# AgnostiqHQ/covalent-ssh-plugin

Hardware: AMD Instinct MI355X
Metric: electrons_per_sec (higher is better)
Workload: dtype n/a; 1 GPU; model=noop-electron-dispatch, global_batch=1, seq_len=0, parallelism=slots1

## Files before the change

### __graft_entry__.py

```python

from __future__ import annotations

import sys
from pathlib import Path

REPO_ROOT = Path(__file__).resolve().parent
if str(REPO_ROOT) not in sys.path:
    sys.path.insert(0, str(REPO_ROOT))


def build() -> None:
    from covalent_ssh_plugin_amd.ops.build import build as build_lib

    lib = build_lib()
    print(f"built {lib}")
    import covalent_ssh_plugin_amd


def smoke() -> None:
    import asyncio
    import ctypes
    import json
    import os
    import tempfile

    import torch

    from covalent_ssh_plugin_amd import SSHExecutor
    from covalent_ssh_plugin_amd.gpu import probe as gpu_probe

    info = gpu_probe.probe(0)
    print("probe:", json.dumps(info))
    assert "gfx950" in info["gcn_arch"], info
    gpu_probe.warmup(0, 50)

    t = torch.randn(1024, 1024, device="cuda:0")
    torch.cuda.synchronize()
    raw = gpu_probe.staged_d2h_bytes(t.data_ptr(), t.numel() * t.element_size())
# ... 58 lines not shown
```

### covalent_ssh_plugin_amd/gpu/probe.py

```python

from __future__ import annotations

import ctypes
import json
import os
from pathlib import Path
from typing import Optional

_LIB_NAME = "libcsp_gpu.so"
_lib: Optional[ctypes.CDLL] = None


class GpuLibError(RuntimeError):
    """The CDNA4 GPU extension is missing or a call into it failed."""


def local_gpu_lib_path() -> str:
    candidate = Path(__file__).resolve().parent.parent / "ops" / _LIB_NAME
    return str(candidate) if candidate.exists() else ""


def load(path: str = "") -> ctypes.CDLL:
    global _lib
    if _lib is not None:
# ... 14 lines not shown
    lib = ctypes.CDLL(lib_path)

    lib.csp_device_count.restype = ctypes.c_int
    lib.csp_probe_json.restype = ctypes.c_int
    lib.csp_probe_json.argtypes = [ctypes.c_int, ctypes.c_char_p, ctypes.c_size_t]
    lib.csp_probe_props_json.restype = ctypes.c_int
    lib.csp_probe_props_json.argtypes = [ctypes.c_int, ctypes.c_char_p, ctypes.c_size_t]
    lib.csp_warmup.restype = ctypes.c_int
    lib.csp_warmup.argtypes = [ctypes.c_int, ctypes.c_int]
    lib.csp_host_alloc.restype = ctypes.c_void_p
    lib.csp_host_alloc.argtypes = [ctypes.c_size_t]
    lib.csp_host_free.restype = ctypes.c_int
    lib.csp_host_free.argtypes = [ctypes.c_void_p]
    lib.csp_staging_get.restype = ctypes.c_void_p
    lib.csp_staging_get.argtypes = [ctypes.c_size_t]
    lib.csp_staging_alloc.restype = ctypes.c_void_p
    lib.csp_staging_alloc.argtypes = [ctypes.c_size_t]
    lib.csp_staging_release_all.restype = ctypes.c_int
    lib.csp_staging_reset.restype = ctypes.c_int
    lib.csp_memcpy_d2h.restype = ctypes.c_int
    lib.csp_memcpy_d2h.argtypes = [ctypes.c_void_p, ctypes.c_void_p, ctypes.c_size_t]
    lib.csp_memcpy_h2d.restype = ctypes.c_int
    lib.csp_memcpy_h2d.argtypes = [ctypes.c_void_p, ctypes.c_void_p, ctypes.c_size_t]
    lib.csp_mem_info.restype = ctypes.c_int
    lib.csp_mem_info.argtypes = [
        ctypes.c_int,
        ctypes.POINTER(ctypes.c_double),
        ctypes.POINTER(ctypes.c_double),
    ]
    lib.csp_last_error.restype = ctypes.c_char_p

    _lib = lib
    return lib


def _check(lib: ctypes.CDLL, rc: int, what: str) -> None:
    if rc != 0:
        err = lib.csp_last_error().decode(errors="replace")
        raise GpuLibError(f"{what} failed (rc={rc}): {err}")


def device_count() -> int:
    lib = load()
    n = lib.csp_device_count()
    if n < 0:
        _check(lib, n, "csp_device_count")
# ... 8 lines not shown


def probe_props(device: int = 0) -> dict:
    lib = load()
    buf = ctypes.create_string_buffer(8192)
    _check(lib, lib.csp_probe_props_json(device, buf, len(buf)), "csp_probe_props_json")
    return json.loads(buf.value.decode())


def mem_info(device: int = 0) -> dict:
    lib = load()
    free_gb = ctypes.c_double()
    total_gb = ctypes.c_double()
    _check(lib, lib.csp_mem_info(device, ctypes.byref(free_gb), ctypes.byref(total_gb)),
           "csp_mem_info")
    return {"hbm_free_gb": free_gb.value, "hbm_total_gb": total_gb.value}


def warmup(device: int = 0, budget_ms: int = 50) -> None:
    lib = load()
    _check(lib, lib.csp_warmup(device, budget_ms), "csp_warmup")


def staged_d2h_bytes(data_ptr: int, nbytes: int) -> bytes:
    lib = load()
    dst = lib.csp_staging_alloc(nbytes)
    if not dst:
        _check(lib, -1, "csp_staging_alloc")
    try:
        _check(
            lib,
            lib.csp_memcpy_d2h(ctypes.c_void_p(dst), ctypes.c_void_p(data_ptr), nbytes),
            "csp_memcpy_d2h",
        )
        return ctypes.string_at(dst, nbytes)
    finally:
        lib.csp_staging_release_all()
```

### covalent_ssh_plugin_amd/ops/build.py

```python

from __future__ import annotations

import os
import shutil
import subprocess
import sys
from pathlib import Path

OPS_DIR = Path(__file__).resolve().parent
SRC = OPS_DIR / "hip" / "csp_gpu.hip"
OUT = OPS_DIR / "libcsp_gpu.so"

HIPCC = shutil.which("hipcc") or "/opt/rocm/bin/hipcc"
ARCH = os.environ.get("PYTORCH_ROCM_ARCH", "gfx950")


def needs_build() -> bool:
    return not OUT.exists() or OUT.stat().st_mtime < SRC.stat().st_mtime


def build(force: bool = False, verbose: bool = True) -> Path:
    if not force and not needs_build():
        return OUT
    cmd = [
        HIPCC,
        f"--offload-arch={ARCH}",
        "-O3",
        "-std=c++17",
        "-fPIC",
        "-shared",
        str(SRC),
        "-o",
        str(OUT),
    ]
    if verbose:
        print("+", " ".join(cmd), file=sys.stderr)
    subprocess.run(cmd, check=True)
    return OUT


if __name__ == "__main__":
    build(force="--force" in sys.argv)
    print(OUT)
```

### covalent_ssh_plugin_amd/ops/hip/csp_gpu.hip

```cpp

#include <hip/hip_runtime.h>
#include <hip/hip_bf16.h>

#include <cstdio>
#include <cstring>
#include <algorithm>
#include <mutex>
#include <vector>
#include <utility>


static thread_local char g_err[512];

static int set_err(const char* what, hipError_t e) {
    snprintf(g_err, sizeof(g_err), "%s: %s", what, hipGetErrorString(e));
    return -1;
}

#define HIP_TRY(expr)                                    \
    do {                                                 \
        hipError_t _e = (expr);                          \
        if (_e != hipSuccess) return set_err(#expr, _e); \
    } while (0)

extern "C" const char* csp_last_error() { return g_err; }


typedef __bf16 bf16x8 __attribute__((ext_vector_type(8)));
// ... 293 lines not shown
    static hipStream_t s = nullptr;
    static std::once_flag once;
    std::call_once(once, [] {
        if (hipStreamCreateWithFlags(&s, hipStreamNonBlocking) != hipSuccess)
            s = nullptr;
    });
    return s;
}

extern "C" int csp_memcpy_d2h(void* dst_host, const void* src_dev, size_t n) {
    hipStream_t s = copy_stream();
    HIP_TRY(hipMemcpyAsync(dst_host, src_dev, n, hipMemcpyDeviceToHost, s));
    HIP_TRY(hipStreamSynchronize(s));
    return 0;
}

extern "C" int csp_memcpy_h2d(void* dst_dev, const void* src_host, size_t n) {
    hipStream_t s = copy_stream();
    HIP_TRY(hipMemcpyAsync(dst_dev, src_host, n, hipMemcpyHostToDevice, s));
    HIP_TRY(hipStreamSynchronize(s));
    return 0;
}

extern "C" int csp_hbm_bench(int device, int variant, size_t bytes, int reps,
                             double* gbps) {
    HIP_TRY(hipSetDevice(device));
    size_t n4 = bytes / sizeof(float4);
    float4 *a = nullptr, *b = nullptr;
    HIP_TRY(hipMalloc(&a, bytes));
    HIP_TRY(hipMalloc(&b, bytes));
    HIP_TRY(hipMemsetAsync(a, 1, bytes));
    float warm_ms = 0.f, ms = 0.f;
    int rc = run_hbm_sweep(a, b, n4, 2, &warm_ms, variant);
    if (rc == 0) rc = run_hbm_sweep(a, b, n4, reps, &ms, variant);
    (void)hipFree(a);
    (void)hipFree(b);
    if (rc != 0) return rc;
    *gbps = (2.0 * (double)bytes * reps / 1.0e9) / ((double)ms / 1000.0);
    return 0;
}

extern "C" int csp_hbm_bench2(int device, int variant, size_t bytes, int reps,
                              int blocks, int pingpong, double* gbps) {
    HIP_TRY(hipSetDevice(device));
    size_t n4 = bytes / sizeof(float4);
    float4 *a = nullptr, *b = nullptr;
// ... 70 lines not shown
```

### covalent_ssh_plugin_amd/remote/stub.py

```python

from __future__ import annotations

import functools
from pathlib import Path
from typing import Optional

_TEMPLATE_PATH = Path(__file__).parent / "stub_template.py"
_WORKER_TEMPLATE_PATH = Path(__file__).parent / "worker_template.py"


@functools.lru_cache(maxsize=2)
def _template_text(path: str) -> str:
    return Path(path).read_text()

DEFAULT_STAGING_THRESHOLD = 64 * 1024 * 1024


def render_stub(
    *,
    remote_result_file: str,
    remote_function_file: str,
    current_remote_workdir: str,
    remote_meta_file: str = "",
    gpu_lib_path: str = "",
    warmup: bool = True,
    staging_threshold: Optional[int] = None,
) -> str:
    text = _template_text(str(_TEMPLATE_PATH))
    thr = DEFAULT_STAGING_THRESHOLD if staging_threshold is None else int(staging_threshold)
    replacements = {
        "__CSP_RESULT_FILE__": remote_result_file,
        "__CSP_FUNCTION_FILE__": remote_function_file,
        "__CSP_WORKDIR__": current_remote_workdir,
        "__CSP_META_FILE__": remote_meta_file,
        "__CSP_GPU_LIB__": gpu_lib_path,
        "__CSP_WARMUP__": repr(bool(warmup)),
        "__CSP_STAGING_THRESHOLD__": str(thr),
    }
    for token, value in replacements.items():
        text = text.replace(token, value)
    return text


@functools.lru_cache(maxsize=64)
def render_worker(
    *,
    gpu_lib_path: str = "",
    warmup: bool = True,
    staging_threshold: Optional[int] = None,
    idle_timeout: float = 0.0,
    isolate: bool = False,
    isolate_preload: str = "torch",
    telemetry_every: int = 0,
) -> str:
    text = _template_text(str(_WORKER_TEMPLATE_PATH))
    thr = DEFAULT_STAGING_THRESHOLD if staging_threshold is None else int(staging_threshold)
    replacements = {
        "__CSP_GPU_LIB__": gpu_lib_path,
        "__CSP_WARMUP__": repr(bool(warmup)),
        "__CSP_STAGING_THRESHOLD__": str(thr),
        "__CSP_IDLE_TIMEOUT__": repr(float(idle_timeout)),
        "__CSP_ISOLATE__": repr(bool(isolate)),
        "__CSP_ISOLATE_PRELOAD__": str(isolate_preload),
        "__CSP_TELEMETRY_EVERY__": str(int(telemetry_every)),
    }
    for token, value in replacements.items():
        text = text.replace(token, value)
    return text
```

### covalent_ssh_plugin_amd/remote/worker_template.py

```python


import json
import os
import struct
import sys
import time

GPU_LIB = "__CSP_GPU_LIB__"
DO_WARMUP = bool(__CSP_WARMUP__)
STAGING_THRESHOLD = int(__CSP_STAGING_THRESHOLD__)
IDLE_TIMEOUT = float(__CSP_IDLE_TIMEOUT__)
ISOLATE = bool(__CSP_ISOLATE__)
ISOLATE_PRELOAD = "__CSP_ISOLATE_PRELOAD__"
TELEMETRY_EVERY = int(__CSP_TELEMETRY_EVERY__)
_last_mem = None

if GPU_LIB:
    GPU_LIB = os.path.abspath(os.path.expanduser(GPU_LIB))


def _resolve_gpu_slot():
    slot = os.environ.get("CSP_GPU_SLOT")
    if slot is None:
        return None
    ambient = os.environ.get("HIP_VISIBLE_DEVICES") or ""
    ids = [x for x in ambient.split(",") if x.strip() != ""]
    if ids:
        os.environ["HIP_VISIBLE_DEVICES"] = ids[int(slot) % len(ids)]
    else:
        os.environ["HIP_VISIBLE_DEVICES"] = slot
    return slot


# ... 28 lines not shown
    if importlib.util.find_spec("torch") is None:
        return
    import torch

    if torch.cuda.is_available():
        torch.cuda.init()


def _load_gpu_lib():
    import ctypes

    _ensure_torch_runtime_first()

    lib = ctypes.CDLL(GPU_LIB)
    lib.csp_probe_json.restype = ctypes.c_int
    lib.csp_probe_json.argtypes = [ctypes.c_int, ctypes.c_char_p, ctypes.c_size_t]
    lib.csp_warmup.restype = ctypes.c_int
    lib.csp_warmup.argtypes = [ctypes.c_int, ctypes.c_int]
    lib.csp_staging_alloc.restype = ctypes.c_void_p
    lib.csp_staging_alloc.argtypes = [ctypes.c_size_t]
    lib.csp_staging_release_all.restype = ctypes.c_int
    lib.csp_memcpy_d2h.restype = ctypes.c_int
    lib.csp_memcpy_d2h.argtypes = [ctypes.c_void_p, ctypes.c_void_p, ctypes.c_size_t]
    lib.csp_mem_info.restype = ctypes.c_int
    lib.csp_mem_info.argtypes = [
        ctypes.c_int,
        ctypes.POINTER(ctypes.c_double),
        ctypes.POINTER(ctypes.c_double),
    ]
    lib.csp_last_error.restype = ctypes.c_char_p
    return lib


def _sample_hbm():
    global _last_mem
    if _gpu_lib is None:
        return
    import ctypes

    free_gb = ctypes.c_double()
    total_gb = ctypes.c_double()
    if _gpu_lib.csp_mem_info(0, ctypes.byref(free_gb), ctypes.byref(total_gb)) == 0:
        _last_mem = {
            "hbm_free_gb": round(free_gb.value, 2),
            "hbm_total_gb": round(total_gb.value, 2),
            "sampled_at_serial": _served,
# ... 2 lines not shown

def _prologue():
    global _gpu_lib, _gpu_info
    import ctypes

    _gpu_lib = _load_gpu_lib()
    buf = ctypes.create_string_buffer(8192)
    rc = _gpu_lib.csp_probe_json(0, buf, len(buf))
    if rc != 0:
        raise RuntimeError(
            "csp_probe_json failed: %s"
            % _gpu_lib.csp_last_error().decode(errors="replace")
        )
    _gpu_info = json.loads(buf.value.decode())
    if DO_WARMUP:
        rc = _gpu_lib.csp_warmup(0, 50)
        if rc != 0:
            raise RuntimeError(
                "csp_warmup failed: %s"
                % _gpu_lib.csp_last_error().decode(errors="replace")
            )


def _stage_result(result, stats, buffers, buffer_meta):
    if "torch" not in sys.modules:
        return result
    import ctypes

    import torch

    lib = _gpu_lib
    if lib is None and GPU_LIB and os.path.exists(GPU_LIB):
        try:
            lib = _load_gpu_lib()
        except Exception:
            lib = None

    def emit_buffer(view, keepalive, dtype, shape):
        buffers.append((view, keepalive))
        buffer_meta.append(
            {"dtype": str(dtype).replace("torch.", ""), "shape": list(shape)}
        )
        return ("__csp_tensor_buffer_v1__", len(buffers) - 1)

    def to_host(t):
        stats["tensors"] += 1
        nbytes = t.numel() * t.element_size()
        stats["bytes"] += nbytes
        if nbytes < STAGING_THRESHOLD:
            return t.cpu() if t.is_cuda else t
        if t.is_cuda:
            if lib is None:
                raise RuntimeError(
                    "CUDA tensor result but the CDNA4 staging library is "
                    "not available on this GPU host"
                )
            src_t = t.contiguous()
            torch.cuda.synchronize()
            dst = lib.csp_staging_alloc(nbytes)
            if not dst:
                raise RuntimeError("csp_staging_alloc failed")
            rc = lib.csp_memcpy_d2h(
                ctypes.c_void_p(dst), ctypes.c_void_p(src_t.data_ptr()), nbytes
            )
            if rc != 0:
                raise RuntimeError("csp_memcpy_d2h failed")
            view = (ctypes.c_char * nbytes).from_address(dst)
            stats["pinned_tensors"] += 1
            stats["mode"] = "pinned"
            return emit_buffer(view, None, src_t.dtype, src_t.shape)
        src_t = t.contiguous()
        view = (ctypes.c_char * nbytes).from_address(src_t.data_ptr())
        if stats["mode"] != "pinned":
            stats["mode"] = "cpu-oob"
        return emit_buffer(view, src_t, src_t.dtype, src_t.shape)

    def walk(obj):
        if isinstance(obj, torch.Tensor):
            return to_host(obj)
        if isinstance(obj, dict):
            return {k: walk(v) for k, v in obj.items()}
        if isinstance(obj, tuple):
            vals = [walk(v) for v in obj]
            return type(obj)(*vals) if hasattr(obj, "_fields") else tuple(vals)
        if isinstance(obj, list):
            return [walk(v) for v in obj]
        return obj

    return walk(result)


def _read_frame(fd, idle_timeout=0.0):
    if idle_timeout > 0:
# ... 135 lines not shown
    _served += 1
    serial = _served
    r, w = os.pipe()
    pid = os.fork()
    if pid == 0:
        os.close(r)
        try:
            import ctypes

            libc = ctypes.CDLL(None, use_errno=True)
            libc.prctl(1, 9, 0, 0, 0)
        except Exception:
            pass
        wrote_reply = False
        try:
            if GPU_LIB and GPU_SLOT is not None and DO_WARMUP:
                _prologue()
            result_blob, meta, buffers = _serve_one(request)
            meta["isolated"] = True
            meta["served"] = serial
            _write_frame(w, pickle.dumps(("R1", result_blob, meta, len(buffers))))
            wrote_reply = True
            for view, _keep in buffers:
                _write_frame(w, view)
        except BaseException as e:
            if not wrote_reply:
                try:
                    blob = pickle.dumps(
                        (None, RuntimeError(f"isolated task failed: {e!r}"))
                    )
                    _write_frame(
                        w,
                        pickle.dumps(
                            ("R1", blob, {"phases_ms": {}, "isolated": True}, 0)
                        ),
                    )
                except BaseException:
                    pass
        os._exit(0)

    os.close(w)
    relayed = 0
    expected = None
    while True:
        frame = _read_frame(r)
        if frame is None or frame == b"":
            break
# ... 46 lines not shown
        sys.exit(3)

    while True:
        frame = _read_frame(0, idle_timeout=IDLE_TIMEOUT)
        if frame is None or frame == b"":
            break
        request = pickle.loads(frame)
        n_arg_bufs = len(request.get("arg_buffers") or [])
        if n_arg_bufs:
            frames = []
            for _ in range(n_arg_bufs):
                f = _read_frame(0)
                if f is None:
                    return
                frames.append(bytearray(f))
            request["_arg_buffer_frames"] = frames
        _write_frame(_proto_fd, pickle.dumps(("A1", request.get("op_id"))))
        if ISOLATE:
            _serve_isolated(request)
            continue
        result_blob, meta, buffers = _serve_one(request)
        _write_frame(_proto_fd, pickle.dumps(("R1", result_blob, meta, len(buffers))))
        for view, _keep in buffers:
            _write_frame(_proto_fd, view)
        del buffers
        if _gpu_lib is not None:
            _gpu_lib.csp_staging_release_all()


if __name__ == "__main__":
    main()
```

### covalent_ssh_plugin_amd/remote/workers.py

```python

from __future__ import annotations

import asyncio
from dataclasses import dataclass, field
from typing import Dict, Optional, Tuple

import cloudpickle

from ..compat import app_log
from ..transport.channel import Channel, ChannelClosed

WorkerKey = Tuple[object, ...]


@dataclass
class WorkerHandle:
    channel: Channel
    startup_meta: dict
    key: WorkerKey

    @property
    def alive(self) -> bool:
        return self.channel.alive

# ... 90 lines not shown
                return extract(obj)
            return obj
        if isinstance(obj, dict):
            return {k: walk(v) for k, v in obj.items()}
        if isinstance(obj, tuple):
            vals = [walk(v) for v in obj]
            return type(obj)(*vals) if hasattr(obj, "_fields") else tuple(vals)
        if isinstance(obj, list):
            return [walk(v) for v in obj]
        return obj

    new_args = walk(list(args))
    new_kwargs = walk(dict(kwargs))
    return new_args, new_kwargs, buffer_meta, buffers


def _reconstruct(result, buffer_meta, buffers):
    import torch

    def build(i: int):
        info = buffer_meta[i]
        dtype = getattr(torch, info["dtype"])
        raw = buffers[i]
        data = raw if isinstance(raw, bytearray) else bytearray(raw)
        t = torch.frombuffer(data, dtype=dtype)
        return t.reshape(info["shape"])

    def walk(obj):
        if (
            isinstance(obj, tuple)
            and len(obj) == 2
            and obj[0] == "__csp_tensor_buffer_v1__"
        ):
            return build(obj[1])
        if isinstance(obj, dict):
            return {k: walk(v) for k, v in obj.items()}
        if isinstance(obj, tuple):
            vals = [walk(v) for v in obj]
            return type(obj)(*vals) if hasattr(obj, "_fields") else tuple(vals)
        if isinstance(obj, list):
            return [walk(v) for v in obj]
        return obj

    return walk(result)


async def run_task(
# ... 67 lines not shown
```

### covalent_ssh_plugin_amd/transport/channel.py

```python

from __future__ import annotations

import asyncio
import struct
from typing import List, Optional


class ChannelClosed(ConnectionError):
    """The remote worker process went away (EOF on its stdout)."""


class Channel:
    def __init__(self, proc: asyncio.subprocess.Process, label: str = "worker"):
        self._proc = proc
        self._label = label
        self._lock = asyncio.Lock()
        self._inflight = 0
        self.loop = asyncio.get_event_loop()

    @property
    def alive(self) -> bool:
        return self._proc.returncode is None

    @property
    def inflight(self) -> int:
        return self._inflight

    async def send_frame(self, payload) -> None:
        if not self.alive:
            raise ChannelClosed(f"{self._label}: process exited")
        view = memoryview(payload).cast("B")
        if view.nbytes <= 64 * 1024:
            self._proc.stdin.write(struct.pack(">Q", view.nbytes) + view.tobytes())
        else:
            self._proc.stdin.write(struct.pack(">Q", view.nbytes))
            self._proc.stdin.write(view)
        await self._proc.stdin.drain()

    async def recv_frame(self, timeout: Optional[float] = None) -> bytes:
        async def _read() -> bytes:
            header = await self._proc.stdout.readexactly(8)
            (length,) = struct.unpack(">Q", header)
            if length == 0:
                return b""
            if length <= (4 << 20):
                return await self._proc.stdout.readexactly(length)
            buf = bytearray(length)
            view = memoryview(buf)
            pos = 0
            while pos < length:
                chunk = await self._proc.stdout.read(length - pos)
                if not chunk:
                    raise asyncio.IncompleteReadError(bytes(view[:pos]), length)
                view[pos : pos + len(chunk)] = chunk
                pos += len(chunk)
            return buf

        try:
            if timeout is None:
                return await _read()
            return await asyncio.wait_for(_read(), timeout=timeout)
        except (asyncio.IncompleteReadError, ConnectionResetError) as e:
            raise ChannelClosed(f"{self._label}: EOF mid-frame") from e

    async def request(self, payload: bytes, timeout: Optional[float] = None) -> bytes:
        async with self._lock:
            await self.send_frame(payload)
            return await self.recv_frame(timeout=timeout)

    def transaction(self):
        return _Transaction(self)


    def _ensure_pump(self) -> None:
        if getattr(self, "_pump_task", None) is None or self._pump_task.done():
            self._waiters: "asyncio.Queue" = asyncio.Queue()
            self._pump_task = asyncio.get_running_loop().create_task(self._pump())

    def _fail_waiters(self, first=None) -> None:
        if first is not None and not first.done():
            first.set_exception(ChannelClosed(f"{self._label}: channel down"))
        waiters = getattr(self, "_waiters", None)
        while waiters is not None and not waiters.empty():
            w, _ = waiters.get_nowait()
            if not w.done():
                try:
# ... 34 lines not shown
        timeout: Optional[float] = None,
    ):
        self._ensure_pump()
        fut = asyncio.get_running_loop().create_future()
        self._inflight += 1
        try:
            async with self._lock:
                self._waiters.put_nowait((fut, reply_frames))
                for frame in request_frames:
                    await self.send_frame(frame)
            if timeout is None:
                return await fut
            return await asyncio.wait_for(fut, timeout=timeout)
        finally:
            self._inflight -= 1

    def kill(self) -> None:
        task = getattr(self, "_pump_task", None)
        if task is not None and not task.done():
            try:
                task.cancel()
            except RuntimeError:
                pass
        if self.alive:
            try:
                self._proc.kill()
            except ProcessLookupError:
                pass

    async def close(self) -> None:
        task = getattr(self, "_pump_task", None)
        if task is not None and not task.done():
            task.cancel()
        if self.loop is not asyncio.get_event_loop() or self.loop.is_closed():
            self.kill()
            return
        if self.alive:
            try:
                self._proc.stdin.write(struct.pack(">Q", 0))
                await self._proc.stdin.drain()
                self._proc.stdin.close()
            except (ConnectionResetError, BrokenPipeError, RuntimeError):
                pass
            try:
                await asyncio.wait_for(self._proc.wait(), timeout=5)
            except asyncio.TimeoutError:
                self._proc.kill()
                await self._proc.wait()


class _Transaction:
    def __init__(self, channel: "Channel"):
        self._channel = channel

    async def __aenter__(self) -> "Channel":
        await self._channel._lock.acquire()
        return self._channel

    async def __aexit__(self, *exc) -> None:
        self._channel._lock.release()


async def open_subprocess_channel(argv: List[str], label: str) -> Channel:
    proc = await asyncio.create_subprocess_exec(
        *argv,
        stdin=asyncio.subprocess.PIPE,
        stdout=asyncio.subprocess.PIPE,
        stderr=None,
        limit=64 * 1024 * 1024,
    )
    return Channel(proc, label=label)
```

### covalent_ssh_plugin_amd/transport/local.py

```python

from __future__ import annotations

import asyncio
import os
import shutil
from pathlib import Path
from typing import Optional, Sequence, Tuple

from .base import CompletedCommand, Transport, TransportConnectError


class LocalTransport(Transport):
    def __init__(self, home: Optional[str] = None):
        self._home = Path(home or os.path.expanduser("~")).resolve()
        self._connected = False
        self.endpoint = f"local:{self._home}"

    @property
    def home(self) -> Path:
        return self._home

    def _resolve(self, remote_path: str) -> Path:
        p = Path(os.path.expanduser(remote_path))
        if not p.is_absolute():
# ... 31 lines not shown
        )
        try:
            stdout, stderr = await asyncio.wait_for(
                proc.communicate(input=input_data), timeout=timeout
            )
        except asyncio.TimeoutError:
            proc.kill()
            await proc.wait()
            raise
        return CompletedCommand(proc.returncode, stdout, stderr)

    async def put_files(self, files: Sequence[Tuple[str, str]]) -> None:
        for local, remote in files:
            dst = self._resolve(remote)
            dst.parent.mkdir(parents=True, exist_ok=True)
            await asyncio.to_thread(shutil.copyfile, local, dst)

    async def get_file(self, remote_path: str, local_path: str) -> None:
        src = self._resolve(remote_path)
        Path(local_path).parent.mkdir(parents=True, exist_ok=True)
        await asyncio.to_thread(shutil.copyfile, src, local_path)

    async def open_channel(self, command: str, env: Optional[dict] = None):
        from .channel import Channel

        full_cmd = self._env_prefix(env) + command
        proc = await asyncio.create_subprocess_exec(
            "bash",
            "-c",
            full_cmd,
            cwd=str(self._home),
            stdin=asyncio.subprocess.PIPE,
            stdout=asyncio.subprocess.PIPE,
            stderr=None,
            limit=64 * 1024 * 1024,
        )
        return Channel(proc, label=f"local-worker")

    async def open_pipe(self, command: str, env: Optional[dict] = None):
        full_cmd = self._env_prefix(env) + command
        return await asyncio.create_subprocess_exec(
            "bash",
            "-c",
            full_cmd,
            cwd=str(self._home),
            stdin=asyncio.subprocess.PIPE,
            stdout=asyncio.subprocess.PIPE,
            stderr=asyncio.subprocess.PIPE,
            limit=4 * 1024 * 1024,
        )

    async def close(self) -> None:
        self._connected = False
```

### covalent_ssh_plugin_amd/transport/openssh.py

```python

from __future__ import annotations

import asyncio
import hashlib
import os
from pathlib import Path
from typing import List, Optional, Sequence, Tuple

from .base import (
    CompletedCommand,
    Transport,
    TransportConnectError,
    make_tar_stream,
)

_SSH_CLIENT_ERR = 255


class OpenSSHTransport(Transport):
    def __init__(
        self,
        hostname: str,
        username: str = "",
        ssh_key_file: str = "",
# ... 129 lines not shown
            with open(local_path, "wb") as f:
                while True:
                    chunk = await proc.stdout.read(1 << 20)
                    if not chunk:
                        break
                    await asyncio.to_thread(f.write, chunk)
        finally:
            await err_task
        rc = await proc.wait()
        if rc != 0:
            try:
                os.remove(local_path)
            except OSError:
                pass
            err = bytes(stderr_acc).decode(errors="replace").strip()
            if rc == _SSH_CLIENT_ERR:
                self._connected = False
                raise TransportConnectError(
                    f"ssh channel to {self.endpoint} failed: {err}"
                )
            raise FileNotFoundError(f"{self.endpoint}:{remote_path}: {err}")

    async def open_channel(self, command: str, env: Optional[dict] = None):
        from .channel import Channel

        argv = self._base_args() + [self.hostname, "--", self._env_prefix(env) + command]
        proc = await asyncio.create_subprocess_exec(
            *argv,
            stdin=asyncio.subprocess.PIPE,
            stdout=asyncio.subprocess.PIPE,
            stderr=None,
            limit=64 * 1024 * 1024,
        )
        return Channel(proc, label=f"worker@{self.endpoint}")

    async def open_pipe(self, command: str, env: Optional[dict] = None):
        argv = self._base_args() + [self.hostname, "--", self._env_prefix(env) + command]
        return await asyncio.create_subprocess_exec(
            *argv,
            stdin=asyncio.subprocess.PIPE,
            stdout=asyncio.subprocess.PIPE,
            stderr=asyncio.subprocess.PIPE,
            limit=4 * 1024 * 1024,
        )

    async def close(self) -> None:
        if not self._connected:
            return
        argv = self._base_args() + ["-O", "exit", self.hostname]
        proc = await asyncio.create_subprocess_exec(
            *argv,
            stdout=asyncio.subprocess.DEVNULL,
            stderr=asyncio.subprocess.DEVNULL,
        )
        await proc.wait()
        self._connected = False
```

### setup.py

```python

from pathlib import Path

from setuptools import find_packages, setup

here = Path(__file__).parent
version = (here / "VERSION").read_text().strip()

setup(
    name="covalent-ssh-plugin-amd",
    version=version,
    description=(
        "MI355X-native Covalent SSH executor: pooled multiplexed SSH dispatch "
        "onto an 8xMI355X node with per-task GPU slots, a CDNA4 warm-up/probe "
        "kernel and hipHostMalloc-pinned result staging"
    ),
    long_description=(here / "README.md").read_text(),
    long_description_content_type="text/markdown",
    packages=find_packages(include=["covalent_ssh_plugin_amd*"]),
    package_data={
        "covalent_ssh_plugin_amd": ["ops/*.so", "ops/hip/*.hip", "remote/stub_template.py"],
    },
    install_requires=[
        line.strip()
        for line in (here / "requirements.txt").read_text().splitlines()
        if line.strip() and not line.startswith("#")
    ],
    extras_require={"covalent": ["covalent>=0.202.0,<1"]},
    entry_points={
        "covalent.executor.executor_plugins": [
            "ssh = covalent_ssh_plugin_amd.ssh",
        ],
    },
    python_requires=">=3.9",
    classifiers=[
        "Programming Language :: Python :: 3.9",
        "Programming Language :: Python :: 3.10",
        "Environment :: GPU",
        "Operating System :: POSIX :: Linux",
    ],
)
```

Baseline: 11390 electrons/s.

## Stream GPU results to worker pipe in chunks and add native pipe reader

Adds a HIP routine that copies a device tensor to host in double-buffered pinned chunks and writes each chunk straight to the worker's output fd, overlapping device-to-host copies with pipe writes. A native C++ IO library and a custom pipe-frame reader replace asyncio StreamReader on the client side, reading frames into preallocated buffers. The aim is to avoid building full staged copies and to cut per-frame copying. The workload is a no-op electron, so these large-buffer paths may rarely run, and the new reader adds protocol complexity on every dispatch.

```diff
diff --git a/__graft_entry__.py b/__graft_entry__.py
--- a/__graft_entry__.py
+++ b/__graft_entry__.py
@@ -10,10 +10,12 @@
 
 
 def build() -> None:
+    from covalent_ssh_plugin_amd.ops.build import IO_OUT
     from covalent_ssh_plugin_amd.ops.build import build as build_lib
 
     lib = build_lib()
     print(f"built {lib}")
+    print(f"built {IO_OUT}")
     import covalent_ssh_plugin_amd
 
 
diff --git a/covalent_ssh_plugin_amd/gpu/probe.py b/covalent_ssh_plugin_amd/gpu/probe.py
--- a/covalent_ssh_plugin_amd/gpu/probe.py
+++ b/covalent_ssh_plugin_amd/gpu/probe.py
@@ -60,6 +60,15 @@
     lib.csp_memcpy_d2h.argtypes = [ctypes.c_void_p, ctypes.c_void_p, ctypes.c_size_t]
     lib.csp_memcpy_h2d.restype = ctypes.c_int
     lib.csp_memcpy_h2d.argtypes = [ctypes.c_void_p, ctypes.c_void_p, ctypes.c_size_t]
+    lib.csp_d2h_stream_fd.restype = ctypes.c_int
+    lib.csp_d2h_stream_fd.argtypes = [
+        ctypes.c_int,
+        ctypes.c_void_p,
+        ctypes.c_size_t,
+        ctypes.c_size_t,
+        ctypes.POINTER(ctypes.c_double),
+        ctypes.POINTER(ctypes.c_double),
+    ]
     lib.csp_mem_info.restype = ctypes.c_int
     lib.csp_mem_info.argtypes = [
         ctypes.c_int,
@@ -114,6 +123,22 @@
     _check(lib, lib.csp_warmup(device, budget_ms), "csp_warmup")
 
 
+STREAM_OK = 0
+STREAM_FAILED_BEFORE_HEADER = 1
+STREAM_FAILED_MID_FRAME = 2
+
+
+def stream_d2h_to_fd(fd: int, data_ptr: int, nbytes: int, chunk_bytes: int = 0) -> dict:
+    lib = load()
+    d2h_ms = ctypes.c_double()
+    write_ms = ctypes.c_double()
+    rc = lib.csp_d2h_stream_fd(
+        fd, ctypes.c_void_p(data_ptr), nbytes, chunk_bytes,
+        ctypes.byref(d2h_ms), ctypes.byref(write_ms),
+    )
+    return {"rc": rc, "d2h_ms": d2h_ms.value, "write_ms": write_ms.value}
+
+
 def staged_d2h_bytes(data_ptr: int, nbytes: int) -> bytes:
     lib = load()
     dst = lib.csp_staging_alloc(nbytes)
diff --git a/covalent_ssh_plugin_amd/ops/build.py b/covalent_ssh_plugin_amd/ops/build.py
--- a/covalent_ssh_plugin_amd/ops/build.py
+++ b/covalent_ssh_plugin_amd/ops/build.py
@@ -6,39 +6,98 @@
 import subprocess
 import sys
 from pathlib import Path
+from typing import List
 
 OPS_DIR = Path(__file__).resolve().parent
 SRC = OPS_DIR / "hip" / "csp_gpu.hip"
 OUT = OPS_DIR / "libcsp_gpu.so"
+IO_SRC = OPS_DIR / "csrc" / "csp_io.cpp"
+IO_HDR = OPS_DIR / "csrc" / "csp_io.h"
+IO_OUT = OPS_DIR / "libcsp_io.so"
 
 HIPCC = shutil.which("hipcc") or "/opt/rocm/bin/hipcc"
 ARCH = os.environ.get("PYTORCH_ROCM_ARCH", "gfx950")
 
 
+def _stale(out: Path, sources: List[Path]) -> bool:
+    if not out.exists():
+        return True
+    built = out.stat().st_mtime
+    return any(built < src.stat().st_mtime for src in sources)
+
+
+def gpu_needs_build() -> bool:
+    return _stale(OUT, [SRC, IO_HDR])
+
+
+def io_needs_build() -> bool:
+    return _stale(IO_OUT, [IO_SRC, IO_HDR])
+
+
 def needs_build() -> bool:
-    return not OUT.exists() or OUT.stat().st_mtime < SRC.stat().st_mtime
+    return gpu_needs_build() or io_needs_build()
+
+
+def _run(cmd: List[str], verbose: bool) -> None:
+    if verbose:
+        print("+", " ".join(cmd), file=sys.stderr)
+    subprocess.run(cmd, check=True)
+
+
+def host_cxx() -> str:
+    for name in (os.environ.get("CXX", ""), "c++", "g++", "clang++"):
+        path = shutil.which(name) if name else None
+        if path:
+            return path
+    return HIPCC
+
+
+def build_io(force: bool = False, verbose: bool = True) -> Path:
+    if not force and not io_needs_build():
+        return IO_OUT
+    _run(
+        [
+            host_cxx(),
+            "-O2",
+            "-std=c++17",
+            "-fPIC",
+            "-shared",
+            "-pthread",
+            str(IO_SRC),
+            "-o",
+            str(IO_OUT),
+        ],
+        verbose,
+    )
+    return IO_OUT
+
+
+def build_gpu(force: bool = False, verbose: bool = True) -> Path:
+    if not force and not gpu_needs_build():
+        return OUT
+    _run(
+        [
+            HIPCC,
+            f"--offload-arch={ARCH}",
+            "-O3",
+            "-std=c++17",
+            "-fPIC",
+            "-shared",
+            str(SRC),
+            "-o",
+            str(OUT),
+        ],
+        verbose,
+    )
+    return OUT
 
 
 def build(force: bool = False, verbose: bool = True) -> Path:
-    if not force and not needs_build():
-        return OUT
-    cmd = [
-        HIPCC,
-        f"--offload-arch={ARCH}",
-        "-O3",
-        "-std=c++17",
-        "-fPIC",
-        "-shared",
-        str(SRC),
-        "-o",
-        str(OUT),
-    ]
-    if verbose:
-        print("+", " ".join(cmd), file=sys.stderr)
-    subprocess.run(cmd, check=True)
-    return OUT
+    build_io(force=force, verbose=verbose)
+    return build_gpu(force=force, verbose=verbose)
 
 
 if __name__ == "__main__":
     build(force="--force" in sys.argv)
     print(OUT)
+    print(IO_OUT)
diff --git a/covalent_ssh_plugin_amd/ops/csrc/csp_io.cpp b/covalent_ssh_plugin_amd/ops/csrc/csp_io.cpp
--- /dev/null
+++ b/covalent_ssh_plugin_amd/ops/csrc/csp_io.cpp
@@ -0,0 +1,32 @@
+
+#include "csp_io.h"
+
+#include <sys/mman.h>
+
+extern "C" {
+
+int csp_io_read_full(int fd, void* dst, size_t n, int timeout_ms) {
+    return csp_io_detail::read_full(fd, dst, n, timeout_ms, nullptr);
+}
+
+int csp_io_write_full(int fd, const void* src, size_t n) {
+    return csp_io_detail::write_full(fd, src, n, nullptr);
+}
+
+void* csp_io_alloc(size_t n) {
+    if (n == 0) return nullptr;
+    void* p = mmap(nullptr, n, PROT_READ | PROT_WRITE,
+                   MAP_PRIVATE | MAP_ANONYMOUS, -1, 0);
+    if (p == MAP_FAILED) return nullptr;
+#ifdef MADV_HUGEPAGE
+    (void)madvise(p, n, MADV_HUGEPAGE);
+#endif
+    return p;
+}
+
+int csp_io_free(void* p, size_t n) {
+    if (!p || n == 0) return 0;
+    return munmap(p, n) == 0 ? 0 : -errno;
+}
+
+}
diff --git a/covalent_ssh_plugin_amd/ops/csrc/csp_io.h b/covalent_ssh_plugin_amd/ops/csrc/csp_io.h
--- /dev/null
+++ b/covalent_ssh_plugin_amd/ops/csrc/csp_io.h
@@ -0,0 +1,104 @@
+
+#pragma once
+
+#include <cerrno>
+#include <csignal>
+#include <cstddef>
+#include <ctime>
+
+#include <poll.h>
+#include <pthread.h>
+#include <unistd.h>
+
+#define CSP_IO_OK 0
+#define CSP_IO_EOF 1
+#define CSP_IO_TIMEOUT 2
+
+namespace csp_io_detail {
+
+static const size_t kMaxPiece = size_t(1) << 30;
+
+static inline int wait_fd(int fd, short events, int timeout_ms) {
+    for (;;) {
+        struct pollfd p;
+        p.fd = fd;
+        p.events = events;
+        p.revents = 0;
+        int rc = poll(&p, 1, timeout_ms);
+        if (rc > 0) return 1;
+        if (rc == 0) return 0;
+        if (errno != EINTR) return -errno;
+    }
+}
+
+static inline int read_full(int fd, void* dst, size_t n, int timeout_ms,
+                            size_t* done) {
+    char* p = static_cast<char*>(dst);
+    size_t got = 0;
+    int rc = CSP_IO_OK;
+    while (got < n) {
+        if (timeout_ms >= 0) {
+            int w = wait_fd(fd, POLLIN, timeout_ms);
+            if (w == 0) { rc = CSP_IO_TIMEOUT; break; }
+            if (w < 0) { rc = w; break; }
+        }
+        size_t want = n - got;
+        if (want > kMaxPiece) want = kMaxPiece;
+        ssize_t r = read(fd, p + got, want);
+        if (r > 0) { got += size_t(r); continue; }
+        if (r == 0) { rc = CSP_IO_EOF; break; }
+        if (errno == EINTR) continue;
+        if (errno == EAGAIN || errno == EWOULDBLOCK) {
+            if (timeout_ms >= 0) continue;
+            int w = wait_fd(fd, POLLIN, -1);
+            if (w < 0) { rc = w; break; }
+            continue;
+        }
+        rc = -errno;
+        break;
+    }
+    if (done) *done = got;
+    return rc;
+}
+
+static inline int write_full(int fd, const void* src, size_t n, size_t* done) {
+    const char* p = static_cast<const char*>(src);
+    size_t put = 0;
+    int rc = CSP_IO_OK;
+
+    sigset_t pipe_set, old_set, pending;
+    sigemptyset(&pipe_set);
+    sigaddset(&pipe_set, SIGPIPE);
+    bool was_pending = false;
+    bool masked = pthread_sigmask(SIG_BLOCK, &pipe_set, &old_set) == 0;
+    if (masked && sigpending(&pending) == 0)
+        was_pending = sigismember(&pending, SIGPIPE) == 1;
+
+    while (put < n) {
+        size_t want = n - put;
+        if (want > kMaxPiece) want = kMaxPiece;
+        ssize_t w = write(fd, p + put, want);
+        if (w >= 0) { put += size_t(w); continue; }
+        if (errno == EINTR) continue;
+        if (errno == EAGAIN || errno == EWOULDBLOCK) {
+            int r = wait_fd(fd, POLLOUT, -1);
+            if (r < 0) { rc = r; break; }
+            continue;
+        }
+        rc = -errno;
+        break;
+    }
+
+    if (masked) {
+        if (rc == -EPIPE && !was_pending) {
+            struct timespec zero = {0, 0};
+            while (sigtimedwait(&pipe_set, nullptr, &zero) < 0 && errno == EINTR) {
+            }
+        }
+        pthread_sigmask(SIG_SETMASK, &old_set, nullptr);
+    }
+    if (done) *done = put;
+    return rc;
+}
+
+}
diff --git a/covalent_ssh_plugin_amd/ops/hip/csp_gpu.hip b/covalent_ssh_plugin_amd/ops/hip/csp_gpu.hip
--- a/covalent_ssh_plugin_amd/ops/hip/csp_gpu.hip
+++ b/covalent_ssh_plugin_amd/ops/hip/csp_gpu.hip
@@ -2,8 +2,11 @@
 #include <hip/hip_runtime.h>
 #include <hip/hip_bf16.h>
 
+#include "../csrc/csp_io.h"
+
 #include <cstdio>
 #include <cstring>
+#include <ctime>
 #include <algorithm>
 #include <mutex>
 #include <vector>
@@ -343,6 +346,123 @@
     return 0;
 }
 
+static void staging_release_one(void* p) {
+    if (!p) return;
+    std::lock_guard<std::mutex> lock(g_staging_mu);
+    for (size_t i = 0; i < g_staging_in_use.size(); ++i) {
+        if (g_staging_in_use[i].first == p) {
+            g_staging_free.push_back(g_staging_in_use[i]);
+            g_staging_in_use.erase(g_staging_in_use.begin() + i);
+            return;
+        }
+    }
+}
+
+static const size_t kStreamChunkDefault = size_t(16) << 20;
+static const int kStreamRing = 2;
+
+#define CSP_STREAM_OK 0
+#define CSP_STREAM_FAILED_BEFORE_HEADER 1
+#define CSP_STREAM_FAILED_MID_FRAME 2
+
+static double mono_ms() {
+    struct timespec ts;
+    clock_gettime(CLOCK_MONOTONIC, &ts);
+    return (double)ts.tv_sec * 1.0e3 + (double)ts.tv_nsec / 1.0e6;
+}
+
+extern "C" int csp_d2h_stream_fd(int fd, const void* src_dev, size_t nbytes,
+                                 size_t chunk_bytes, double* d2h_ms,
+                                 double* write_ms) {
+    if (d2h_ms) *d2h_ms = 0.0;
+    if (write_ms) *write_ms = 0.0;
+    if (chunk_bytes == 0) chunk_bytes = kStreamChunkDefault;
+    if (chunk_bytes > nbytes) chunk_bytes = nbytes;
+    const size_t nchunks = nbytes ? (nbytes + chunk_bytes - 1) / chunk_bytes : 0;
+    const int ring = nchunks < (size_t)kStreamRing ? (int)nchunks : kStreamRing;
+
+    unsigned char header[8];
+    for (int i = 0; i < 8; ++i)
+        header[i] = (unsigned char)((unsigned long long)nbytes >> (8 * (7 - i)));
+
+    hipStream_t s = copy_stream();
+    void* buf[kStreamRing] = {nullptr, nullptr};
+    hipEvent_t ev_start[kStreamRing] = {nullptr, nullptr};
+    hipEvent_t ev_done[kStreamRing] = {nullptr, nullptr};
+    const char* src = static_cast<const char*>(src_dev);
+    bool header_out = false;
+    bool copies_issued = false;
+    double t_d2h = 0.0, t_write = 0.0;
+    int rc = CSP_STREAM_OK;
+
+    auto fail_hip = [&](const char* what, hipError_t e) {
+        set_err(what, e);
+        rc = header_out ? CSP_STREAM_FAILED_MID_FRAME : CSP_STREAM_FAILED_BEFORE_HEADER;
+    };
+    auto fail_io = [&](const char* what, int io_rc) {
+        snprintf(g_err, sizeof(g_err), "%s: %s", what, strerror(-io_rc));
+        rc = header_out ? CSP_STREAM_FAILED_MID_FRAME : CSP_STREAM_FAILED_BEFORE_HEADER;
+    };
+    auto issue = [&](size_t i) -> bool {
+        const int slot = (int)(i % kStreamRing);
+        const size_t off = i * chunk_bytes;
+        const size_t len = std::min(chunk_bytes, nbytes - off);
+        hipError_t e = hipEventRecord(ev_start[slot], s);
+        if (e == hipSuccess)
+            e = hipMemcpyAsync(buf[slot], src + off, len, hipMemcpyDeviceToHost, s);
+        if (e == hipSuccess) e = hipEventRecord(ev_done[slot], s);
+        copies_issued = true;
+        if (e != hipSuccess) { fail_hip("stream chunk copy", e); return false; }
+        return true;
+    };
+    auto timed_write = [&](const void* p, size_t n) -> bool {
+        size_t done = 0;
+        const double t0 = mono_ms();
+        int io_rc = csp_io_detail::write_full(fd, p, n, &done);
+        t_write += mono_ms() - t0;
+        if (done > 0) header_out = true;
+        if (io_rc != CSP_IO_OK) { fail_io("stream write", io_rc); return false; }
+        return true;
+    };
+
+    for (int k = 0; k < ring && rc == CSP_STREAM_OK; ++k) {
+        buf[k] = csp_staging_alloc(chunk_bytes);
+        if (!buf[k]) { rc = CSP_STREAM_FAILED_BEFORE_HEADER; break; }
+        hipError_t e = hipEventCreate(&ev_start[k]);
+        if (e == hipSuccess) e = hipEventCreate(&ev_done[k]);
+        if (e != hipSuccess) fail_hip("hipEventCreate", e);
+    }
+
+    if (rc == CSP_STREAM_OK && nchunks > 0) issue(0);
+    if (rc == CSP_STREAM_OK && nchunks > 0) {
+        hipError_t e = hipEventSynchronize(ev_done[0]);
+        if (e != hipSuccess) fail_hip("hipEventSynchronize", e);
+    }
+    if (rc == CSP_STREAM_OK) timed_write(header, sizeof(header));
+
+    for (size_t i = 0; i < nchunks && rc == CSP_STREAM_OK; ++i) {
+        const int slot = (int)(i % kStreamRing);
+        if (i + 1 < nchunks && !issue(i + 1)) break;
+        hipError_t e = hipEventSynchronize(ev_done[slot]);
+        if (e != hipSuccess) { fail_hip("hipEventSynchronize", e); break; }
+        float ms = 0.f;
+        if (hipEventElapsedTime(&ms, ev_start[slot], ev_done[slot]) == hipSuccess)
+            t_d2h += ms;
+        const size_t off = i * chunk_bytes;
+        if (!timed_write(buf[slot], std::min(chunk_bytes, nbytes - off))) break;
+    }
+
+    if (copies_issued && rc != CSP_STREAM_OK) (void)hipStreamSynchronize(s);
+    for (int k = 0; k < kStreamRing; ++k) {
+        if (ev_start[k]) (void)hipEventDestroy(ev_start[k]);
+        if (ev_done[k]) (void)hipEventDestroy(ev_done[k]);
+        staging_release_one(buf[k]);
+    }
+    if (d2h_ms) *d2h_ms = t_d2h;
+    if (write_ms) *write_ms = t_write;
+    return rc;
+}
+
 extern "C" int csp_hbm_bench(int device, int variant, size_t bytes, int reps,
                              double* gbps) {
     HIP_TRY(hipSetDevice(device));
diff --git a/covalent_ssh_plugin_amd/remote/stub.py b/covalent_ssh_plugin_amd/remote/stub.py
--- a/covalent_ssh_plugin_amd/remote/stub.py
+++ b/covalent_ssh_plugin_amd/remote/stub.py
@@ -14,6 +14,8 @@
     return Path(path).read_text()
 
 DEFAULT_STAGING_THRESHOLD = 64 * 1024 * 1024
+
+STREAM_CHUNK_BYTES = 16 * 1024 * 1024
 
 
 def render_stub(
@@ -59,6 +61,7 @@
         "__CSP_GPU_LIB__": gpu_lib_path,
         "__CSP_WARMUP__": repr(bool(warmup)),
         "__CSP_STAGING_THRESHOLD__": str(thr),
+        "__CSP_STREAM_CHUNK__": str(STREAM_CHUNK_BYTES),
         "__CSP_IDLE_TIMEOUT__": repr(float(idle_timeout)),
         "__CSP_ISOLATE__": repr(bool(isolate)),
         "__CSP_ISOLATE_PRELOAD__": str(isolate_preload),
diff --git a/covalent_ssh_plugin_amd/remote/worker_template.py b/covalent_ssh_plugin_amd/remote/worker_template.py
--- a/covalent_ssh_plugin_amd/remote/worker_template.py
+++ b/covalent_ssh_plugin_amd/remote/worker_template.py
@@ -9,6 +9,7 @@
 GPU_LIB = "__CSP_GPU_LIB__"
 DO_WARMUP = bool(__CSP_WARMUP__)
 STAGING_THRESHOLD = int(__CSP_STAGING_THRESHOLD__)
+STREAM_CHUNK = int(__CSP_STREAM_CHUNK__)
 IDLE_TIMEOUT = float(__CSP_IDLE_TIMEOUT__)
 ISOLATE = bool(__CSP_ISOLATE__)
 ISOLATE_PRELOAD = "__CSP_ISOLATE_PRELOAD__"
@@ -83,6 +84,15 @@
     lib.csp_staging_release_all.restype = ctypes.c_int
     lib.csp_memcpy_d2h.restype = ctypes.c_int
     lib.csp_memcpy_d2h.argtypes = [ctypes.c_void_p, ctypes.c_void_p, ctypes.c_size_t]
+    lib.csp_d2h_stream_fd.restype = ctypes.c_int
+    lib.csp_d2h_stream_fd.argtypes = [
+        ctypes.c_int,
+        ctypes.c_void_p,
+        ctypes.c_size_t,
+        ctypes.c_size_t,
+        ctypes.POINTER(ctypes.c_double),
+        ctypes.POINTER(ctypes.c_double),
+    ]
     lib.csp_mem_info.restype = ctypes.c_int
     lib.csp_mem_info.argtypes = [
         ctypes.c_int,
@@ -131,6 +141,32 @@
             )
 
 
+class _DeferredCuda:
+
+    def __init__(self, lib, ptr, nbytes):
+        self.lib = lib
+        self.ptr = ptr
+        self.nbytes = nbytes
+
+
+def _send_buffer(fd, view):
+    if not isinstance(view, _DeferredCuda):
+        _write_frame(fd, view)
+        return
+    import ctypes
+
+    rc = view.lib.csp_d2h_stream_fd(
+        fd, ctypes.c_void_p(view.ptr), view.nbytes, STREAM_CHUNK, None, None
+    )
+    if rc != 0:
+        sys.stderr.write(
+            "csp worker: csp_d2h_stream_fd failed (rc=%d): %s\n"
+            % (rc, view.lib.csp_last_error().decode(errors="replace"))
+        )
+        sys.stderr.flush()
+        os._exit(4)
+
+
 def _stage_result(result, stats, buffers, buffer_meta):
     if "torch" not in sys.modules:
         return result
@@ -166,18 +202,10 @@
                 )
             src_t = t.contiguous()
             torch.cuda.synchronize()
-            dst = lib.csp_staging_alloc(nbytes)
-            if not dst:
-                raise RuntimeError("csp_staging_alloc failed")
-            rc = lib.csp_memcpy_d2h(
-                ctypes.c_void_p(dst), ctypes.c_void_p(src_t.data_ptr()), nbytes
-            )
-            if rc != 0:
-                raise RuntimeError("csp_memcpy_d2h failed")
-            view = (ctypes.c_char * nbytes).from_address(dst)
+            view = _DeferredCuda(lib, src_t.data_ptr(), nbytes)
             stats["pinned_tensors"] += 1
             stats["mode"] = "pinned"
-            return emit_buffer(view, None, src_t.dtype, src_t.shape)
+            return emit_buffer(view, src_t, src_t.dtype, src_t.shape)
         src_t = t.contiguous()
         view = (ctypes.c_char * nbytes).from_address(src_t.data_ptr())
         if stats["mode"] != "pinned":
@@ -359,7 +387,7 @@
             _write_frame(w, pickle.dumps(("R1", result_blob, meta, len(buffers))))
             wrote_reply = True
             for view, _keep in buffers:
-                _write_frame(w, view)
+                _send_buffer(w, view)
         except BaseException as e:
             if not wrote_reply:
                 try:
@@ -452,7 +480,7 @@
         result_blob, meta, buffers = _serve_one(request)
         _write_frame(_proto_fd, pickle.dumps(("R1", result_blob, meta, len(buffers))))
         for view, _keep in buffers:
-            _write_frame(_proto_fd, view)
+            _send_buffer(_proto_fd, view)
         del buffers
         if _gpu_lib is not None:
             _gpu_lib.csp_staging_release_all()
diff --git a/covalent_ssh_plugin_amd/remote/workers.py b/covalent_ssh_plugin_amd/remote/workers.py
--- a/covalent_ssh_plugin_amd/remote/workers.py
+++ b/covalent_ssh_plugin_amd/remote/workers.py
@@ -136,7 +136,7 @@
         info = buffer_meta[i]
         dtype = getattr(torch, info["dtype"])
         raw = buffers[i]
-        data = raw if isinstance(raw, bytearray) else bytearray(raw)
+        data = bytearray(raw) if isinstance(raw, bytes) else raw
         t = torch.frombuffer(data, dtype=dtype)
         return t.reshape(info["shape"])
 
diff --git a/covalent_ssh_plugin_amd/transport/channel.py b/covalent_ssh_plugin_amd/transport/channel.py
--- a/covalent_ssh_plugin_amd/transport/channel.py
+++ b/covalent_ssh_plugin_amd/transport/channel.py
@@ -2,17 +2,183 @@
 from __future__ import annotations
 
 import asyncio
+import os
 import struct
 from typing import List, Optional
 
+from . import native_io
+
 
 class ChannelClosed(ConnectionError):
     """The remote worker process went away (EOF on its stdout)."""
 
 
+class _PipeFrameReader(asyncio.Protocol):
+
+    FLOW_LIMIT = 8 << 20
+
+    def __init__(self, loop: asyncio.AbstractEventLoop):
+        self._loop = loop
+        self._buf = bytearray()
+        self._waiter: Optional[asyncio.Future] = None
+        self._eof = False
+        self._transport = None
+        self._flow_paused = False
+        self._held = False
+        self._sink: Optional[memoryview] = None
+        self._sink_pos = 0
+
+    def connection_made(self, transport) -> None:
+        self._transport = transport
+
+    def data_received(self, data: bytes) -> None:
+        sink = self._sink
+        if sink is not None:
+            pos = self._sink_pos
+            room = len(sink) - pos
+            if len(data) <= room:
+                sink[pos : pos + len(data)] = data
+                self._sink_pos = pos + len(data)
+            else:
+                chunk = memoryview(data)
+                sink[pos:] = chunk[:room]
+                self._sink_pos = len(sink)
+                self._buf += chunk[room:]
+        else:
+            self._buf += data
+            if len(self._buf) > self.FLOW_LIMIT and not self._flow_paused:
+                self._flow_paused = True
+                self._apply_pause()
+        self._wake()
+
+    def eof_received(self) -> None:
+        self._eof = True
+        self._wake()
+
+    def connection_lost(self, exc) -> None:
+        self._eof = True
+        self._wake()
+
+    def _apply_pause(self) -> None:
+        t = self._transport
+        if t is None or t.is_closing():
+            return
+        if self._flow_paused or self._held:
+            t.pause_reading()
+        else:
+            t.resume_reading()
+
+    def _flow_resume(self) -> None:
+        if self._flow_paused:
+            self._flow_paused = False
+            self._apply_pause()
+
+    def hold(self) -> None:
+        self._held = True
+        self._apply_pause()
+
+    def release(self) -> None:
+        self._held = False
+        self._apply_pause()
+
+    def _wake(self) -> None:
+        w = self._waiter
+        if w is not None and not w.done():
+            w.set_result(None)
+
+    async def _wait(self) -> None:
+        if self._waiter is not None:
+            raise RuntimeError("channel read side has two concurrent readers")
+        self._waiter = self._loop.create_future()
+        try:
+            await self._waiter
+        finally:
+            self._waiter = None
+
+    def at_eof(self) -> bool:
+        return self._eof
+
+    def fileno(self) -> Optional[int]:
+        t = self._transport
+        if t is None or t.is_closing():
+            return None
+        pipe = t.get_extra_info("pipe")
+        return None if pipe is None else pipe.fileno()
+
+    async def readexactly(self, n: int) -> bytes:
+        buf = self._buf
+        while len(buf) < n:
+            if self._eof:
+                partial = bytes(buf)
+                buf.clear()
+                raise asyncio.IncompleteReadError(partial, n)
+            self._flow_resume()
+            await self._wait()
+        if len(buf) == n:
+            data = bytes(buf)
+            buf.clear()
+        else:
+            data = bytes(memoryview(buf)[:n])
+            del buf[:n]
+        if self._flow_paused and len(buf) <= self.FLOW_LIMIT:
+            self._flow_resume()
+        return data
+
+    def take_into(self, view: memoryview) -> int:
+        k = min(len(self._buf), len(view))
+        if k:
+            with memoryview(self._buf) as m:
+                view[:k] = m[:k]
+            del self._buf[:k]
+            if self._flow_paused and len(self._buf) <= self.FLOW_LIMIT:
+                self._flow_resume()
+        return k
+
+    async def read_into(self, view: memoryview) -> None:
+        n = len(view)
+        pos = self.take_into(view)
+        if pos == n:
+            return
+        self._sink, self._sink_pos = view, pos
+        try:
+            while self._sink_pos < n:
+                if self._eof:
+                    raise asyncio.IncompleteReadError(b"", n)
+                self._flow_resume()
+                await self._wait()
+        finally:
+            self._sink = None
+
+    def close(self) -> None:
+        t = self._transport
+        if t is not None:
+            try:
+                t.close()
+            except RuntimeError:
+                pass
+
+
+def _native_fill(fd: int, buf: bytearray, pos: int, nbytes: int, timeout_ms: int) -> int:
+    try:
+        return native_io.read_full(fd, buf, nbytes, timeout_ms, offset=pos)
+    finally:
+        os.close(fd)
+
+
 class Channel:
-    def __init__(self, proc: asyncio.subprocess.Process, label: str = "worker"):
+    large_frame_threshold = 4 << 20
+    large_frame_idle_timeout = 300.0
+    large_frame_huge_pages = True
+
+    def __init__(
+        self,
+        proc: asyncio.subprocess.Process,
+        label: str = "worker",
+        reader: Optional[_PipeFrameReader] = None,
+    ):
         self._proc = proc
+        self._reader = reader
+        self._broken = False
         self._label = label
         self._lock = asyncio.Lock()
         self._inflight = 0
@@ -20,7 +186,7 @@
 
     @property
     def alive(self) -> bool:
-        return self._proc.returncode is None
+        return self._proc.returncode is None and not self._broken
 
     @property
     def inflight(self) -> int:
@@ -37,31 +203,87 @@
             self._proc.stdin.write(view)
         await self._proc.stdin.drain()
 
+    async def _recv_large(self, length: int):
+        reader = self._reader
+        buf = native_io.alloc_buffer(length) if self.large_frame_huge_pages else None
+        if buf is None:
+            buf = bytearray(length)
+        view = memoryview(buf).cast("B")
+        native = native_io.load() is not None and reader.fileno() is not None
+        loop = asyncio.get_running_loop()
+        complete = False
+        if native:
+            reader.hold()
+        try:
+            if not native:
+                await reader.read_into(view)
+                complete = True
+                return buf
+            pos = reader.take_into(view)
+            if pos < length:
+                if reader.at_eof():
+                    raise asyncio.IncompleteReadError(b"", length)
+                fd = os.dup(reader.fileno())
+                rc = await loop.run_in_executor(
+                    None, _native_fill, fd, buf, pos, length - pos,
+                    int(self.large_frame_idle_timeout * 1000),
+                )
+                if rc == native_io.EOF:
+                    raise asyncio.IncompleteReadError(b"", length)
+                if rc != native_io.OK:
+                    raise ChannelClosed(
+                        f"{self._label}: large-frame read failed: "
+                        f"{native_io.strerror(rc)}"
+                    )
+            complete = True
+            return buf
+        finally:
+            if complete:
+                if native:
+                    reader.release()
+            else:
+                self._broken = True
+                self.kill()
+
     async def recv_frame(self, timeout: Optional[float] = None) -> bytes:
         async def _read() -> bytes:
-            header = await self._proc.stdout.readexactly(8)
+            reader = self._reader
+            if reader is None:
+                return await self._read_stream_reader()
+            header = await reader.readexactly(8)
             (length,) = struct.unpack(">Q", header)
             if length == 0:
                 return b""
-            if length <= (4 << 20):
-                return await self._proc.stdout.readexactly(length)
-            buf = bytearray(length)
-            view = memoryview(buf)
-            pos = 0
-            while pos < length:
-                chunk = await self._proc.stdout.read(length - pos)
-                if not chunk:
-                    raise asyncio.IncompleteReadError(bytes(view[:pos]), length)
-                view[pos : pos + len(chunk)] = chunk
-                pos += len(chunk)
-            return buf
-
+            if length <= self.large_frame_threshold:
+                return await reader.readexactly(length)
+            return await self._recv_large(length)
+
+        if self._broken:
+            raise ChannelClosed(f"{self._label}: channel abandoned mid-frame")
         try:
             if timeout is None:
                 return await _read()
             return await asyncio.wait_for(_read(), timeout=timeout)
         except (asyncio.IncompleteReadError, ConnectionResetError) as e:
             raise ChannelClosed(f"{self._label}: EOF mid-frame") from e
+
+    async def _read_stream_reader(self) -> bytes:
+        header = await self._proc.stdout.readexactly(8)
+        (length,) = struct.unpack(">Q", header)
+        if length == 0:
+            return b""
+        if length <= self.large_frame_threshold:
+            return await self._proc.stdout.readexactly(length)
+        buf = bytearray(length)
+        view = memoryview(buf)
+        pos = 0
+        while pos < length:
+            chunk = await self._proc.stdout.read(length - pos)
+            if not chunk:
+                raise asyncio.IncompleteReadError(bytes(view[:pos]), length)
+            view[pos : pos + len(chunk)] = chunk
+            pos += len(chunk)
+        return buf
 
     async def request(self, payload: bytes, timeout: Optional[float] = None) -> bytes:
         async with self._lock:
@@ -142,11 +364,13 @@
                 task.cancel()
             except RuntimeError:
                 pass
-        if self.alive:
+        if self._proc.returncode is None:
             try:
                 self._proc.kill()
             except ProcessLookupError:
                 pass
+        if self._reader is not None:
+            self._reader.close()
 
     async def close(self) -> None:
         task = getattr(self, "_pump_task", None)
@@ -167,6 +391,8 @@
             except asyncio.TimeoutError:
                 self._proc.kill()
                 await self._proc.wait()
+        if self._reader is not None:
+            self._reader.close()
 
 
 class _Transaction:
@@ -181,12 +407,31 @@
         self._channel._lock.release()
 
 
+async def spawn_channel_process(argv: List[str], label: str, **kwargs) -> Channel:
+    loop = asyncio.get_running_loop()
+    r_fd, w_fd = os.pipe()
+    try:
+        proc = await asyncio.create_subprocess_exec(
+            *argv,
+            stdin=asyncio.subprocess.PIPE,
+            stdout=w_fd,
+            stderr=None,
+            limit=64 * 1024 * 1024,
+            **kwargs,
+        )
+    except BaseException:
+        os.close(r_fd)
+        raise
+    finally:
+        os.close(w_fd)
+    reader = _PipeFrameReader(loop)
+    try:
+        await loop.connect_read_pipe(lambda: reader, os.fdopen(r_fd, "rb", 0))
+    except BaseException:
+        proc.kill()
+        raise
+    return Channel(proc, label=label, reader=reader)
+
+
 async def open_subprocess_channel(argv: List[str], label: str) -> Channel:
-    proc = await asyncio.create_subprocess_exec(
-        *argv,
-        stdin=asyncio.subprocess.PIPE,
-        stdout=asyncio.subprocess.PIPE,
-        stderr=None,
-        limit=64 * 1024 * 1024,
-    )
-    return Channel(proc, label=label)
+    return await spawn_channel_process(argv, label)
diff --git a/covalent_ssh_plugin_amd/transport/local.py b/covalent_ssh_plugin_amd/transport/local.py
--- a/covalent_ssh_plugin_amd/transport/local.py
+++ b/covalent_ssh_plugin_amd/transport/local.py
@@ -77,20 +77,12 @@
         await asyncio.to_thread(shutil.copyfile, src, local_path)
 
     async def open_channel(self, command: str, env: Optional[dict] = None):
-        from .channel import Channel
+        from .channel import spawn_channel_process
 
         full_cmd = self._env_prefix(env) + command
-        proc = await asyncio.create_subprocess_exec(
-            "bash",
-            "-c",
-            full_cmd,
-            cwd=str(self._home),
-            stdin=asyncio.subprocess.PIPE,
-            stdout=asyncio.subprocess.PIPE,
-            stderr=None,
-            limit=64 * 1024 * 1024,
+        return await spawn_channel_process(
+            ["bash", "-c", full_cmd], label="local-worker", cwd=str(self._home)
         )
-        return Channel(proc, label=f"local-worker")
 
     async def open_pipe(self, command: str, env: Optional[dict] = None):
         full_cmd = self._env_prefix(env) + command
diff --git a/covalent_ssh_plugin_amd/transport/native_io.py b/covalent_ssh_plugin_amd/transport/native_io.py
--- /dev/null
+++ b/covalent_ssh_plugin_amd/transport/native_io.py
@@ -0,0 +1,110 @@
+
+from __future__ import annotations
+
+import ctypes
+import os
+import weakref
+from pathlib import Path
+from typing import Optional
+
+_LIB_NAME = "libcsp_io.so"
+
+OK = 0
+EOF = 1
+TIMEOUT = 2
+
+_lib: Optional[ctypes.CDLL] = None
+_tried = False
+force_absent = False
+
+
+def local_io_lib_path() -> str:
+    candidate = Path(__file__).resolve().parent.parent / "ops" / _LIB_NAME
+    return str(candidate) if candidate.exists() else ""
+
+
+def load(path: str = "") -> Optional[ctypes.CDLL]:
+    global _lib, _tried
+    if force_absent:
+        return None
+    if _lib is not None or (_tried and not path):
+        return _lib
+    _tried = True
+    lib_path = path or local_io_lib_path()
+    if not lib_path:
+        return None
+    try:
+        lib = ctypes.CDLL(lib_path, use_errno=True)
+    except OSError:
+        return None
+    lib.csp_io_read_full.restype = ctypes.c_int
+    lib.csp_io_read_full.argtypes = [
+        ctypes.c_int, ctypes.c_void_p, ctypes.c_size_t, ctypes.c_int,
+    ]
+    lib.csp_io_write_full.restype = ctypes.c_int
+    lib.csp_io_write_full.argtypes = [ctypes.c_int, ctypes.c_void_p, ctypes.c_size_t]
+    lib.csp_io_alloc.restype = ctypes.c_void_p
+    lib.csp_io_alloc.argtypes = [ctypes.c_size_t]
+    lib.csp_io_free.restype = ctypes.c_int
+    lib.csp_io_free.argtypes = [ctypes.c_void_p, ctypes.c_size_t]
+    _lib = lib
+    return lib
+
+
+def _address(buf, offset: int, nbytes: int) -> tuple:
+    view = memoryview(buf).cast("B")
+    if offset < 0 or nbytes < 0 or offset + nbytes > view.nbytes:
+        raise ValueError("range outside the buffer")
+    if nbytes == 0:
+        return 0, view
+    window = view[offset : offset + nbytes]
+    carrier = (ctypes.c_char * nbytes).from_buffer(window)
+    return ctypes.addressof(carrier), (carrier, window)
+
+
+def read_full(fd: int, buf, nbytes: int, timeout_ms: int, offset: int = 0) -> int:
+    lib = load()
+    if lib is None:
+        raise RuntimeError(f"{_LIB_NAME} is not built")
+    addr, keep = _address(buf, offset, nbytes)
+    rc = lib.csp_io_read_full(fd, addr, nbytes, timeout_ms)
+    del keep
+    return rc
+
+
+def write_full(fd: int, buf, nbytes: Optional[int] = None, offset: int = 0) -> int:
+    lib = load()
+    if lib is None:
+        raise RuntimeError(f"{_LIB_NAME} is not built")
+    if nbytes is None:
+        nbytes = memoryview(buf).nbytes - offset
+    view = memoryview(buf).cast("B")
+    if nbytes == 0:
+        return lib.csp_io_write_full(fd, None, 0)
+    window = view[offset : offset + nbytes]
+    if window.readonly:
+        return lib.csp_io_write_full(fd, bytes(window), nbytes)
+    carrier = (ctypes.c_char * nbytes).from_buffer(window)
+    return lib.csp_io_write_full(fd, ctypes.addressof(carrier), nbytes)
+
+
+def alloc_buffer(nbytes: int):
+    lib = load()
+    if lib is None or nbytes <= 0:
+        return None
+    addr = lib.csp_io_alloc(nbytes)
+    if not addr:
+        return None
+    arr = (ctypes.c_ubyte * nbytes).from_address(addr)
+    weakref.finalize(arr, lib.csp_io_free, addr, nbytes)
+    return arr
+
+
+def strerror(rc: int) -> str:
+    if rc == OK:
+        return "ok"
+    if rc == EOF:
+        return "end of file"
+    if rc == TIMEOUT:
+        return "timed out"
+    return os.strerror(-rc)
diff --git a/covalent_ssh_plugin_amd/transport/openssh.py b/covalent_ssh_plugin_amd/transport/openssh.py
--- a/covalent_ssh_plugin_amd/transport/openssh.py
+++ b/covalent_ssh_plugin_amd/transport/openssh.py
@@ -175,17 +175,10 @@
             raise FileNotFoundError(f"{self.endpoint}:{remote_path}: {err}")
 
     async def open_channel(self, command: str, env: Optional[dict] = None):
-        from .channel import Channel
+        from .channel import spawn_channel_process
 
         argv = self._base_args() + [self.hostname, "--", self._env_prefix(env) + command]
-        proc = await asyncio.create_subprocess_exec(
-            *argv,
-            stdin=asyncio.subprocess.PIPE,
-            stdout=asyncio.subprocess.PIPE,
-            stderr=None,
-            limit=64 * 1024 * 1024,
-        )
-        return Channel(proc, label=f"worker@{self.endpoint}")
+        return await spawn_channel_process(argv, label=f"worker@{self.endpoint}")
 
     async def open_pipe(self, command: str, env: Optional[dict] = None):
         argv = self._base_args() + [self.hostname, "--", self._env_prefix(env) + command]
diff --git a/setup.py b/setup.py
--- a/setup.py
+++ b/setup.py
@@ -18,7 +18,7 @@
     long_description_content_type="text/markdown",
     packages=find_packages(include=["covalent_ssh_plugin_amd*"]),
     package_data={
-        "covalent_ssh_plugin_amd": ["ops/*.so", "ops/hip/*.hip", "remote/stub_template.py"],
+        "covalent_ssh_plugin_amd": ["ops/*.so", "ops/hip/*.hip", "ops/csrc/*.cpp", "ops/csrc/*.h", "remote/stub_template.py"],
     },
     install_requires=[
         line.strip()
```

Measured after the change: 11710 electrons/s (median of 6 runs). +2.8%, better.
